# pku-lab-1806-llm/lab-1806-vec-db

Measured on AMD Instinct MI355X. Metric: queries/sec at recall@10, Gist1M d=960 (Flat brute force, L2Sqr, k=10), higher is better.
Workload: dtype f32 (int8 lower-bound filter pass); 1 GPU; flat_knn_gist1m; rows=1000000, dim=960, k=10, dist=L2Sqr, parallelism=single GPU, steps_in_flight=1, queries_per_corpus_pass=128

## Files before the change

### lab_1806_vec_db_amd/csrc/api.hip

```cpp
#include <algorithm>
#include <cmath>
#include <cstring>

#include "ctx.hpp"
#include "pq_hnsw.hpp"

using namespace vdb;

static thread_local std::string g_last_error;
void vdb::set_last_error(const std::string &m) { g_last_error = m; }
void vdb::require_gpu() {
    int cnt = 0;
    hipError_t e = hipGetDeviceCount(&cnt);
    if (e != hipSuccess || cnt <= 0)
        throw Error(VDB_ERR_NOGPU, std::string("no usable HIP device (libvdbhip has no CPU fallback): ") +
                                       hipGetErrorString(e));
}

void vdb::merge_topk_dev(Index &ix, const void *d_dists, const void *d_ids, const void *d_counts, uint64_t stride_d,
                           uint64_t stride_i, uint64_t stride_c, uint64_t n_shards, uint64_t nq, uint64_t k,
                           void *d_out_idx, void *d_out_dist, void *d_out_count, void *stream) {
    VDB_REQUIRE(d_dists && d_ids && d_counts && d_out_idx && d_out_dist && d_out_count, "null argument");
    VDB_REQUIRE(k >= 1 && k <= 1024, "k must be in 1..1024");
    VDB_REQUIRE(nq <= 65535 && n_shards <= 65535, "too many queries or shards for one call");
// ... 434 lines not shown
        ivf_set_q8((int)value);
    else if (n == "hnsw_build_gpu")
        hnsw_set_build_gpu((int)value);
    else if (n == "hnsw_pool_cap")
        hnsw_set_pool_cap((int)value);
    else if (n == "pq_adc_fast")
        pq_set_adc_fast((int)value);
    else if (n == "pq_sample16")
        pq_set_adc16_sample((int)value);
    else if (n == "pq_adc16")
        pq_set_adc16((int)value);
    else if (n == "pq_adc8_sliced")
        pq_set_adc8_sliced((int)value);
    else if (n == "flat_sample_thin")
        mfma_set_sample_thin((int)value);
    else if (n == "flat_gemm_tw")
        gemm_set_tw((int)value);
    else if (n == "flat_gemm_nt")
        gemm_set_nt((int)value);
    else if (n == "flat_gemm_zigzag")
        gemm_set_zigzag((int)value);
    else if (n == "flat_gemm_block_rows") {
        VDB_REQUIRE(value >= 0, "flat_gemm_block_rows must be >= 0");
        gemm_set_block_rows((uint64_t)value);
    }
    else if (n == "flat_gemm_stagger")
        gemm_set_stagger((int)value);
    else if (n == "flat_gemm_debug")
        idx->ix.flat_gemm_debug = (int)value;
    else if (n == "flat_tail")
        idx->ix.flat_tail_mode = (int)value;
    else if (n == "flat_tail_lb_nw")
        flat_tail_lb_set_nw((int)value);
    else if (n == "flat_small")
        idx->ix.flat_small_mode = (int)value;
    else if (n == "flat_small_max_rows")
        idx->ix.flat_small_max_rows = (uint64_t)value;
    else if (n == "flat_half")
        idx->ix.flat_half_mode = (int)value;
    else if (n == "flat_i8")
        idx->ix.flat_i8_mode = (int)value;
    else if (n == "flat_i8_rows") {
        VDB_REQUIRE(value >= 64 && value <= 8192 && value % 64 == 0, "flat_i8_rows must be a multiple of 64 in [64, 8192]");
        idx->ix.flat_i8_kprime = (uint32_t)value;
    }
    else if (n == "debug_alloc_fail_over")
        devbuf_fail_over() = (size_t)value;
    else if (n == "flat_i8_unit_min")
        idx->ix.flat_i8_unit_min = (int)value;
    else if (n == "flat_i8_full")
        idx->ix.flat_i8_full = (int)value;
    else if (n == "flat_i8_refine") {
        idx->ix.flat_i8_refine = (int)value;
        idx->ix.i8_refine_on = 0;
        idx->ix.i8_refine_calls = 0;
    }
    else if (n == "flat_i8_second")
        idx->ix.flat_i8_second = (int)value;
    else if (n == "flat_i8_stats") {
        idx->ix.flat_i8_stats = (int)value;
        for (auto &h : idx->ix.i8_rounds_hist) h = 0;
        idx->ix.i8_hits_sum = 0;
        idx->ix.i8_hits_max = 0;
        idx->ix.i8_stat_queries = 0;
    }
    else if (n == "flat_i8_hits") {
        VDB_REQUIRE(value >= 256 && value <= 4096, "flat_i8_hits must be in [256, 4096]");
        idx->ix.flat_i8_hits = (uint32_t)value;
    }
    else if (n == "flat_gemm8_sample_res")
        gemm8_set_sample_res((int)value);
    else if (n == "flat_gemm8_nt")
        gemm8_set_nt((int)value);
    else if (n == "flat_gemm8_kc")
        gemm8_set_kc((int)value);
    else if (n == "flat_gemm8_burst")
        gemm8_set_burst((int)value);
    else if (n == "flat_gemm8_res")
        gemm8_set_res((int)value);
    else if (n == "flat_gemm8_coop")
        gemm8_set_coop((int)value);
    else if (n == "flat_gemm8_grid")
        gemm8_set_grid((int)value);
    else if (n == "flat_gemm_coop")
        gemm_set_coop((int)value);
    else if (n == "flat_half_kmul") {
        VDB_REQUIRE(value >= 1 && value <= 64, "flat_half_kmul must be in [1, 64]");
        idx->ix.flat_half_kmul = (uint32_t)value;
    }
    else
        throw Error(VDB_ERR_INVALID, "unknown parameter " + n);
    VDB_API_END
}
int vdb_index_prepare(vdb_index *idx, int all_tiers) {
    VDB_API_BEGIN
    VDB_REQUIRE(idx, "null index");
    require_gpu();
// ... 15 lines not shown
        *out = idx->ix.fallback_count.load();
    else if (n == "flat_half_queries")
        *out = idx->ix.half_queries.load();
    else if (n == "flat_half_redo")
        *out = idx->ix.half_redo.load();
    else if (n == "flat_half_valid")
        *out = idx->ix.half_m.valid ? 1 : 0;
    else if (n == "flat_gemm_coop_sets")
        *out = gemm_last_coop();
    else if (n == "flat_gemm8_coop_sets")
        *out = gemm8_last_coop();
    else if (n == "flat_i8_queries")
        *out = idx->ix.i8_queries.load();
    else if (n == "flat_i8_redo")
        *out = idx->ix.i8_redo.load();
    else if (n == "flat_i8_valid")
        *out = idx->ix.i8_m.valid ? 1 : 0;
    else if (n.rfind("flat_i8_rounds_", 0) == 0 && n.size() == 16 && n[15] >= '0' && n[15] <= '8')
        *out = idx->ix.i8_rounds_hist[n[15] - '0'].load();
    else if (n == "mirror_alloc_failures")
        *out = idx->ix.mirror_alloc_failures.load();
    else if (n == "flat_i8_second_queries")
        *out = idx->ix.i8_second_queries.load();
    else if (n == "flat_i8_second_redo")
        *out = idx->ix.i8_second_redo.load();
    else if (n == "flat_i8_hits_sum")
        *out = idx->ix.i8_hits_sum.load();
    else if (n == "flat_i8_hits_max")
        *out = idx->ix.i8_hits_max.load();
    else if (n == "flat_i8_stat_queries")
        *out = idx->ix.i8_stat_queries.load();
    else if (n == "flat_i8_rows_walked")
        *out = idx->ix.i8_rows_walked.load();
    else if (n == "flat_bf16_mirror")
        *out = idx->ix.tiled_built ? 1 : 0;
    else if (n == "hnsw_heap_walk_queries")
        *out = idx->ix.hnsw.heap_walk_queries.load();
    else if (n == "hnsw_half_dropped")
        *out = idx->ix.hnsw.last_half_dropped.load();
    else if (n == "ivf_last_offers")
        *out = idx->ix.ivf.last_offers.load();
    else if (n == "ivf_last_rows_fetched_q8")
        *out = idx->ix.ivf.last_rows_fetched_q8.load();
    else if (n == "ivf_last_kept_q8")
        *out = idx->ix.ivf.last_kept_q8.load();
    else if (n == "ivf_last_kept")
        *out = idx->ix.ivf.last_kept.load();
    else if (n == "pq_adc16_queries")
        *out = idx->ix.pq.adc16_queries.load();
    else if (n == "pq_adc16_redo")
        *out = idx->ix.pq.adc16_redo.load();
    else if (n == "flat_i8_refine_queries")
        *out = idx->ix.i8_refine_queries.load();
    else if (n == "flat_i8_refine_on")
        *out = (uint64_t)idx->ix.i8_refine_on.load();
    else if (n == "pq_q8_overflow")
        *out = idx->ix.pq.q8_overflow.load();
    else if (n == "pq_q8_short")
        *out = idx->ix.pq.q8_short.load();
    else if (n == "pq_q8_hits_sum")
        *out = idx->ix.pq.q8_hits_sum.load();
    else if (n == "pq_q8_hits_max")
        *out = idx->ix.pq.q8_hits_max.load();
    else if (n == "hbm_bytes_per_row")
        *out = idx->ix.hbm_bytes_per_row();
    else
// ... 508 lines not shown
```

### lab_1806_vec_db_amd/csrc/index.hip

```cpp
#include "index.hpp"

#include <algorithm>
#include <cmath>
#include <cstring>

namespace vdb {

Index::Index(int dev, uint64_t d, int ds, bool u8) : device(dev), dim(d), dist(ds), elem_u8(u8) {
#ifndef VDB_HOST_SANITIZER_BUILD
    use_device();
    hipDeviceProp_t prop;
    VDB_HIP(hipGetDeviceProperties(&prop, dev));
    num_cu = prop.multiProcessorCount > 0 ? prop.multiProcessorCount : 256;
    std::string arch = prop.gcnArchName;
    if (arch.rfind("gfx950", 0) != 0)
        throw Error(4, "libvdbhip is built for gfx950 (MI355X) only; device reports " + arch);
#endif
}

std::unique_ptr<Workspace> Index::acquire_ws() {
    use_device();
    {
        std::lock_guard<std::mutex> g(ws_mu);
        if (!ws_free.empty()) {
// ... 564 lines not shown
            launch_mfma_pack_queries_nh(d_q, (uint32_t)nq, (uint32_t)nq_pad, (uint32_t)dim, 8, ws.qfrag_g.as<float>(), s);
        }
    }
    if (i8_second) {
        launch_i8_tau_from_dk(d_dk_hint, (uint32_t)nq, (uint32_t)nq_pad, d_qoff, ws.qsq.as<float>(), xsq_max, i8_mu_norm, (uint32_t)dim, cosine,
                              d_tau, s);
    } else {
        if (i8)
            launch_flat_gemm8_sample(d_tiled_i8.p, n, (uint32_t)dim, ws.qfrag_g.p, d_qscale, (uint32_t)ngroups, d_rowc_i8.as<float>(), s_step,
                                     ws.dense.as<float>(), ld_s, num_cu, s, unit_min ? 1 : 0);
        else if (gemm)
            launch_flat_gemm_sample(xt, n, (uint32_t)dim, ws.qfrag_g.as<float>(), d_qmul, (uint32_t)ngroups,
                                    d_sq.as<float>(), cosine, s_step, ws.dense.as<float>(), ld_s, num_cu, s);
        else
            launch_flat_mfma_sample(d_tiled.as<float>(), n, (uint32_t)dim, ws.qfrag.as<float>(), (uint32_t)nbatch,
                                    d_sq.as<float>(), cosine, s_step, ws.dense.as<float>(), ld_s, num_cu, s);
        if (n_s <= select_tau_max_n()) {
            launch_select_tau(ws.dense.as<float>(), ld_s, (uint32_t)n_s, (uint32_t)nq_pad, (uint32_t)nq, s_rank, d_tau, s);
        } else {
            const uint32_t cap_s = topk_capacity(s_rank);
            launch_topk_dense(ws.dense.as<float>(), ld_s, n_s, (uint32_t)nq_pad, s_rank, ws.lists.as<uint64_t>(), s);
            launch_topk_merge(ws.lists.as<uint64_t>(), nl_s, cap_s, (uint32_t)nq_pad, s_rank, ws.keys_a.as<uint64_t>(), s);
            launch_extract_tau(ws.keys_a.as<uint64_t>(), cap_s, (uint32_t)nq_pad, s_rank, d_tau, s);
        }
        if (nq_pad > nq && n_s > select_tau_max_n())
            VDB_HIP(hipMemsetD32Async(reinterpret_cast<hipDeviceptr_t>(d_tau + nq), (int)0xFF800000u, nq_pad - nq, s));
    }
    uint64_t *d_cand = ws.lists.as<uint64_t>();
    uint32_t *d_sync = d_hits + nq_pad;
    if (!half && !i8) VDB_HIP(hipMemsetAsync(d_hits, 0, (nq_pad + sync_words) * sizeof(uint32_t), s));
    const uint64_t hbm_passes = gemm ? ngroups : (nbatch + mfma_share() - 1) / mfma_share();
    {
        std::lock_guard<std::mutex> g(pass_mu);
        if (pass_ev_valid) VDB_HIP(hipStreamWaitEvent(s, pass_ev, 0));
    }
    prof_begin(ws, i8 ? "flat_i8" : (half ? "flat_half" : "flat_mfma"),
               double(hbm_passes) * double(n) * dim * (i8 ? 1 : (half ? sizeof(uint16_t) : sizeof(float))));
    if (i8)
        launch_flat_gemm8_filter(d_tiled_i8.p, n, (uint32_t)dim, ws.qfrag_g.p, d_qscale, (uint32_t)ngroups, d_rowc_i8.as<float>(), d_tau,
                                 d_cand, d_hits, CAND_CAP, flat_gemm_debug, num_cu, s,
                                 i8_second ? CAND_CAP : std::max<uint32_t>(64u, s_step * s_rank));
    else if (gemm)
        launch_flat_gemm_filter(xt, n, (uint32_t)dim, ws.qfrag_g.as<float>(), d_qmul, (uint32_t)ngroups,
                                d_sq.as<float>(), cosine, d_tau, d_cand, d_hits, CAND_CAP, flat_gemm_debug, num_cu, s);
    else
        launch_flat_mfma_filter(d_tiled.as<float>(), n, (uint32_t)dim, ws.qfrag.as<float>(), (uint32_t)nbatch,
                                d_sq.as<float>(), cosine, d_tau, d_cand, d_hits, CAND_CAP, d_sync, num_cu, s);
    prof_end(ws);
    {
        std::lock_guard<std::mutex> g(pass_mu);
        if (!pass_ev) VDB_HIP(hipEventCreateWithFlags(&pass_ev, hipEventDisableTiming));
        VDB_HIP(hipEventRecord(pass_ev, s));
        pass_ev_valid = true;
    }
    SplitErr se;
    if (half) {
        se.qerr = d_qerr;
        se.dx_abs = half_dx_abs;
        se.dx_rel = half_dx_rel;
    }
    if (i8) {
        se.qoff = d_qoff;
        se.mu_norm = i8_mu_norm;
    }
    if (i8 || (flat_tail_mode != 1 && !elem_u8 && flat_tail64_supported((uint32_t)dim, kprime, ksel))) {
        FlatTailArgs t{};
        t.cand = d_cand;
        t.cap = CAND_CAP;
        t.cnt = d_hits;
        t.kprime = kprime;
        t.ksel = ksel;
        t.kstride = (uint32_t)k;
        t.X = d_rows.as<float>();
        t.dim = (uint32_t)dim;
        t.Q = d_q;
        t.metric = cosine ? MET_COSINE : MET_L2_DIRECT;
        t.xsq = d_sq.as<float>();
        t.qsq = ws.qsq.as<float>();
        t.n_rows = n;
        t.xsq_max = xsq_max;
        t.xsq_min_pos = xsq_min_pos;
        t.cosine = cosine;
        t.se = se;
        t.id_offset = id_offset;
        bool refine = false;
        if (i8 && !i8_second && nq >= 64 && flat_i8_refine != 1) {
            bool on = flat_i8_refine == 2;
            if (flat_i8_refine == 0 && i8_refine_on.load() != 0) on = (i8_refine_calls.fetch_add(1) % 32u) != 31u;
            refine = on && ensure_rows_h(ws);
        }
        const size_t st_off = (nq + 15) & ~size_t(15);
        const bool want_stats = i8 && flat_i8_stats;
        t.flags = static_cast<uint8_t *>(ws.pinned(want_stats ? st_off + nq * sizeof(uint32_t) : nq));
        if (want_stats) t.qstat = reinterpret_cast<uint32_t *>(t.flags + st_off);
        p.stats = want_stats;
        p.refined = refine;
        if (refine) {
            launch_flat_refine_half(d_rows_h.as<uint16_t>(), (uint32_t)dim, half_sx(), half_dx_abs, half_dx_rel, cosine, d_q, d_sq.as<float>(),
                                    ws.qsq.as<float>(), d_qoff, d_cand, CAND_CAP, d_hits, (uint32_t)nq, CAND_CAP, s);
            i8_refine_queries += nq;
        }
        t.out_idx = d_idx;
        t.out_dist = d_dist;
        t.out_count = d_cnt;
        t.tau = d_tau;
        if (i8 && i8_second && nq <= 96 && flat_i8_full != 1) {
            ws.keys_b.reserve(nq * size_t(CAND_CAP) * sizeof(uint64_t));
            launch_flat_full_lb(t, (uint32_t)nq, ws.keys_b.as<uint64_t>(), ws.keys_c.as<uint64_t>(), s);
        } else if (i8)
            launch_flat_tail_lb(t, (uint32_t)nq, s);
        else
            launch_flat_tail64(t, (uint32_t)nq, s);
    } else {
        launch_topk_merge_counted(d_cand, CAND_CAP, d_hits, (uint32_t)nq, kprime, ws.keys_a.as<uint64_t>(), s);
        rerank_rows((uint32_t)dim, d_q, (uint32_t)nq, cosine ? MET_COSINE : MET_L2_DIRECT, d_sq.as<float>(),
                      ws.qsq.as<float>(), ws.keys_a.as<uint64_t>(), ws.keys_b.as<uint64_t>(), kprime, capp, s);
        launch_topk_merge(ws.keys_b.as<uint64_t>(), 1, capp, (uint32_t)nq, ksel, ws.keys_c.as<uint64_t>(), s);
        launch_flat_finish(ws.keys_c.as<uint64_t>(), capk, ws.keys_a.as<uint64_t>(), capp, (uint32_t)nq, ksel, (uint32_t)k, kprime,
                           n, ws.qsq.as<float>(), xsq_max, xsq_min_pos, cosine, (uint32_t)dim, se, d_hits, CAND_CAP, id_offset,
                           static_cast<uint8_t *>(ws.pinned(nq)), d_idx, d_dist, d_cnt, s);
    }
    p.active = true;
    p.half = half;
    p.i8 = i8;
    p.i8_second = i8_second;
    p.kprime = kprime;
// ... 13 lines not shown
    const uint64_t nq = p.nq, k = p.k;
    const uint8_t *flags = static_cast<const uint8_t *>(ws.pinned(nq));
    VDB_SYNC(s);
    std::vector<uint64_t> redo;
    for (uint64_t q = 0; q < nq; q++)
        if (flags[q] & 1u) redo.push_back(q);
    if (p.half) {
        half_queries += nq;
        half_redo += redo.size();
    }
    if (p.i8 && p.i8_second) {
        i8_second_queries += nq;
        i8_second_redo += redo.size();
    }
    const bool try_second = p.i8 && !p.i8_second && flat_i8_second != 1 && !redo.empty();
    if (p.i8 && !p.i8_second) {
        i8_queries += nq;
        if (!try_second) i8_redo += redo.size();
        if (flat_i8_refine == 0 && nq >= 64) {
            uint64_t rs = 0;
            for (uint64_t q = 0; q < nq; q++) rs += std::min<uint32_t>(flags[q] >> 1, 32u);
            const double mean_rounds = double(rs) / double(nq);
            if (!p.refined) {
                const int was = i8_refine_on.load();
                const int now = was ? (mean_rounds >= 4.0 ? 1 : 0) : (mean_rounds >= 6.0 ? 1 : 0);
                if (now != was) {
                    i8_refine_on = now;
                    i8_refine_calls = 0;
                }
            }
        }
        if (p.stats) {
            const uint32_t *qs = reinterpret_cast<const uint32_t *>(flags + ((nq + 15) & ~size_t(15)));
            uint64_t hs = 0, hm = 0;
            for (uint64_t q = 0; q < nq; q++) {
                const uint32_t r = qs[q] & 0xFFu, h = qs[q] >> 8;
                i8_rounds_hist[r < 8 ? r : 8] += 1;
                hs += h;
                hm = std::max<uint64_t>(hm, h);
            }
            i8_hits_sum += hs;
            i8_stat_queries += nq;
            uint64_t cur = i8_hits_max.load();
            while (hm > cur && !i8_hits_max.compare_exchange_weak(cur, hm)) {
            }
        }
    }
    if (redo.empty()) return 0;
    if (!p.half && !p.i8) fallback_count += redo.size();
    const uint64_t nr = redo.size();
    DevBuf rx, rq, rqs, ri, rd, rc, rdk;
    rx.reserve(nr * sizeof(uint64_t));
    rq.reserve(nr * dim * sizeof(float));
    rqs.reserve(nr * sizeof(float));
    ri.reserve(nr * k * sizeof(uint64_t));
    rd.reserve(nr * k * sizeof(float));
    rc.reserve(nr * sizeof(uint64_t));
    VDB_HIP(hipMemcpyAsync(rx.p, redo.data(), nr * sizeof(uint64_t), hipMemcpyHostToDevice, s));
    launch_gather_rows_f32(p.d_q, rx.as<uint64_t>(), nr, (uint32_t)dim, rq.as<float>(), s);
    launch_gather_rows_f32(ws.qsq.as<float>(), rx.as<uint64_t>(), nr, 1, rqs.as<float>(), s);
    if (try_second) {
        rdk.reserve(nr * sizeof(float));
        launch_gather_dk(p.d_dist, p.d_cnt, rx.as<uint64_t>(), nr, (uint32_t)k, p.ksel, rdk.as<float>(), s);
    }
    VDB_HIP(hipMemsetAsync(ri.p, 0, nr * k * sizeof(uint64_t), s));
    VDB_HIP(hipMemsetAsync(rd.p, 0, nr * k * sizeof(float), s));
    VDB_SYNC(s);
    if (try_second)
        i8_redo += flat_knn_device(ws, rq.as<float>(), nr, k, ri.as<uint64_t>(), rd.as<float>(), rc.as<uint64_t>(), true, 0, true, rdk.as<float>());
    else if (p.i8)
        flat_knn_device(ws, rq.as<float>(), nr, k, ri.as<uint64_t>(), rd.as<float>(), rc.as<uint64_t>(), true, 0, false);
    else if (p.half)
        flat_knn_device(ws, rq.as<float>(), nr, k, ri.as<uint64_t>(), rd.as<float>(), rc.as<uint64_t>(), false, p.kprime);
// ... 79 lines not shown
```

### lab_1806_vec_db_amd/csrc/index.hpp

```cpp
#pragma once
#include <algorithm>
#include <atomic>
#include <cmath>
#include <cstdlib>
#include <functional>
#include <map>
#include <memory>
#include <mutex>
#include <string>
#include <vector>

#include "common.hpp"
#include "kernels.hpp"

namespace vdb {

inline bool devbuf_efence() {
    static const bool on = [] {
        const char *e = std::getenv("VDB_EFENCE");
        return e && e[0] == '1';
    }();
    return on;
}
inline std::atomic<size_t> &devbuf_fail_over() {
// ... 229 lines not shown
    bool ensure_tiled(Workspace &ws);
    void prepare_flat(bool all_tiers);
    uint64_t hbm_bytes_per_row() const;
    DevBuf d_tiled_h, d_half_err;
    int half_exp = 0;
    float half_dx_abs = 0.0f, half_dx_rel = 0.0f;
    int flat_half_mode = 0;
    uint32_t flat_half_kmul = 4;
    std::atomic<uint64_t> half_queries{0}, half_redo{0};
    void half_refresh(Workspace &ws, uint64_t n_old, uint64_t n_new);
    RowMirror half_m{mirror_alloc_failures, {&d_tiled_h}};
    bool i8_defers_half() const;
    bool ensure_half(Workspace &ws);
    float half_sx() const { return std::ldexp(1.0f, 13 - half_exp); }
    DevBuf d_tiled_i8, d_rowc_i8, d_mu_i8;
    RowMirror i8_m{mirror_alloc_failures, {&d_tiled_i8, &d_rowc_i8}};
    uint64_t i8_mu_rows = 0;
    float i8_l1 = 0.0f, i8_l2 = 0.0f, i8_mu_norm = 0.0f;
    int flat_i8_mode = 0;
    uint32_t flat_i8_kprime = 2048;
    int flat_i8_full = 0;
    int flat_i8_refine = 0;
    std::atomic<int> i8_refine_on{0};
    std::atomic<uint32_t> i8_refine_calls{0};
    std::atomic<uint64_t> i8_refine_queries{0};
    int flat_i8_unit_min = 0;
    int flat_i8_second = 0;
    std::atomic<uint64_t> i8_second_queries{0}, i8_second_redo{0};
    uint32_t flat_i8_hits = 1024;
    std::atomic<uint64_t> i8_queries{0}, i8_redo{0};
    int flat_i8_stats = 0;
    std::atomic<uint64_t> i8_rounds_hist[9] = {};
    std::atomic<uint64_t> i8_hits_sum{0}, i8_hits_max{0}, i8_stat_queries{0};
    std::atomic<uint64_t> i8_rows_walked{0};
    bool i8_applicable(uint32_t ksel) const;
    bool ensure_i8(Workspace &ws);
    void build_i8(Workspace &ws);
    DevBuf d_rows_h;
    RowMirror rows_h_m{mirror_alloc_failures, {&d_rows_h}};
    int rows_h_exp = 0;
    bool ensure_rows_h(Workspace &ws);
    DevBuf d_rows_q8, d_q8_scale, d_q8_err;
    RowMirror rows_q8_m{mirror_alloc_failures, {&d_rows_q8, &d_q8_scale, &d_q8_err}};
    bool ensure_rows_q8(Workspace &ws);
    std::vector<float> h_sq;
    float xsq_max = 0.0f;
    float xsq_min_pos = 3.4e38f;
    mutable std::vector<float> h_rows;
    mutable bool host_valid = true;
    mutable std::mutex host_mu;
    int flat_mode = 0;
    int flat_gemm_mode = 0;
    int flat_gemm_debug = 0;
    int flat_tail_mode = 0;
    int flat_small_mode = 0;
    uint64_t flat_small_max_rows = 16384;
    bool flat_small_applies(uint64_t nq, uint64_t k) const;
    void flat_small_device(Workspace &ws, const float *q, uint64_t nq, uint64_t k, uint64_t *o_idx, float *o_dist, uint64_t *o_cnt);
    std::atomic<uint64_t> fallback_count{0};
    PQState pq;
    HNSWState hnsw;
    IVFState ivf;

    std::mutex ws_mu;
    std::vector<std::unique_ptr<Workspace>> ws_free;
    std::mutex pass_mu;
    hipEvent_t pass_ev = nullptr;
    bool pass_ev_valid = false;
    bool prof_on = false;
    std::mutex prof_mu;
    std::map<std::string, ProfEntry> prof;

    Index(int dev, uint64_t d, int ds, bool u8 = false);
    ~Index() {
        if (pass_ev) (void)hipEventDestroy(pass_ev);
    }
    void use_device() const {
#ifndef VDB_HOST_SANITIZER_BUILD
        VDB_HIP(hipSetDevice(device));
#endif
    }
    std::unique_ptr<Workspace> acquire_ws();
    void release_ws(std::unique_ptr<Workspace> ws);
    const float *host_rows() const;

    void add_rows(const void *rows, uint64_t count, bool on_device);
    void swap_remove(uint64_t i);

    void prof_begin(Workspace &ws, const char *name, double bytes);
    void prof_end(Workspace &ws);
    void prof_collect(Workspace &ws);

    uint64_t flat_knn_device(Workspace &ws, const float *d_q, uint64_t nq, uint64_t k, uint64_t *d_idx, float *d_dist,
                         uint64_t *d_cnt, bool allow_half = true, uint32_t kprime_min = 0, bool allow_i8 = true,
                         const float *d_dk_hint = nullptr);
    void flat_knn_enqueue(Workspace &ws, const float *d_q, uint64_t nq, uint64_t k, uint64_t *d_idx, float *d_dist, uint64_t *d_cnt,
                          bool allow_half, uint32_t kprime_min, FlatPending &p, bool allow_i8 = true, const float *d_dk_hint = nullptr);
    uint64_t flat_knn_finish(Workspace &ws, FlatPending &p);
    void flat_sorted_device(Workspace &ws, const float *d_q, uint64_t nq, uint64_t ksel, uint64_t k, uint64_t *d_idx,
                            float *d_dist, uint64_t *d_cnt);
    void scan_rows(uint64_t nrows, uint32_t d, const float *Q, uint32_t nq, int metric, const float *xsq, const float *qsq, float *out,
// ... 20 lines not shown
```

### lab_1806_vec_db_amd/csrc/k_exact.hip

```cpp
#include <algorithm>
#include <atomic>
#include <cstdio>
#include <cstdlib>
#include <vector>

#include "common.hpp"
#include "kernels.hpp"

#pragma clang fp contract(off)

namespace vdb {

enum Fold : int { FOLD_L2 = 0, FOLD_DOT = 1 };

template <int FOLD>
__device__ __forceinline__ float fold1(float acc, float x, float q) {
    if (FOLD == FOLD_L2) {
        float df = x - q;
        float sq = df * df;
        return acc + sq;
    } else {
        float p = x * q;
        return acc + p;
    }
// ... 767 lines not shown
    VDB_HIP(hipGetLastError());
}

#define TAIL_LB_AUTO_NW(nq) 40
template <int NW>
__device__ __forceinline__ uint64_t block_top64_above(const uint64_t *__restrict__ src, uint32_t total, uint64_t (*sbest)[64], uint64_t above) {
    const uint32_t lane = threadIdx.x & 63, wave = threadIdx.x >> 6;
    const uint32_t batches = (total + 255) / 256;
    uint64_t best = PAIR_NONE;
    for (uint32_t bt = wave; bt < batches; bt += NW) {
        uint64_t r[4];
#pragma unroll
        for (int u = 0; u < 4; u++) {
            const uint32_t i = (bt * 4 + u) * 64 + lane;
            const uint64_t v = i < total ? src[i] : PAIR_NONE;
            r[u] = v > above ? v : PAIR_NONE;
        }
        const uint64_t tau = __shfl(best, 63);
        uint64_t lo = r[0] < r[1] ? r[0] : r[1], lo2 = r[2] < r[3] ? r[2] : r[3];
        lo = lo < lo2 ? lo : lo2;
        if (__ballot(lo < tau) == 0) continue;
        bitonic_sort_from<2, 4>(r, lane);
        const uint64_t a = merge64(r[0], r[1], lane), b = merge64(r[2], r[3], lane);
        best = merge64(best, merge64(a, b, lane), lane);
    }
    sbest[wave][lane] = best;
    __syncthreads();
    if (wave != 0) return PAIR_NONE;
    uint64_t m = sbest[0][lane];
#pragma unroll
    for (int w = 1; w < NW; w++) m = merge64(m, sbest[w][lane], lane);
    return m;
}
__device__ __forceinline__ uint8_t flat_certify_lb(uint64_t ek, float kappa, uint32_t q, const FlatTailArgs &a) {
    if (ek == PAIR_NONE) return 1;
    const float dk = f32_from_orderable(uint32_t(ek >> 32));
    if (a.cosine) {
        const float qs = a.qsq[q], qn = sqrtf(qs);
        const bool plain = a.xsq_min_pos >= 1e-30f && qs >= 1e-30f && qs <= 1e30f && sqrtf(a.xsq_min_pos) * qn > 1e-9f;
        const float nr = 2.0f + 2.0f * a.se.mu_norm;
        float lower = 0.5f * (kappa + a.se.qoff[q]);
        lower = lower - 4.0f * 5.9604645e-8f * fabsf(lower) - float(2 * a.dim + 16) * 5.9604645e-8f * 1.01f - 2.0f * 5.9604645e-8f * nr * nr;
        return (plain && dk < lower) ? 0 : 1;
    }
    const float qn = sqrtf(a.qsq[q]);
    const float rx = fminf(sqrtf(a.xsq_max), (qn + sqrtf(fmaxf(dk, 0.0f))) * 1.001f);
    const float nr = rx + qn + 2.0f * a.se.mu_norm;
    float lower = kappa + a.se.qoff[q];
    lower = lower - float(a.dim + 8) * 5.9604645e-8f * 1.01f * fabsf(lower) - 4.0f * 5.9604645e-8f * nr * nr;
    return dk < lower ? 0 : 1;
}
template <int FOLD, int NW, int PCD>
__global__ __launch_bounds__(NW * 64, PCD ? 4 : 1) void k_flat_tail_lb(FlatTailArgs a) {
    constexpr bool PC = PCD != 0;
    static_assert(NW == 8 || NW == 4 || NW == 2 || NW == 1, "a stage covers the 64 keys of a round");
    static_assert(!PC || NW == 4, "producer / consumer fold: four waves");
    constexpr int RW = 64 / NW, NP = RW / 8;
    constexpr int DEPTH = PC ? PCD : (NW == 8 ? 8 : (NW == 4 ? 4 : (NW == 2 ? 3 : 2)));
    extern __shared__ float4 ftl_smem[];
    __shared__ uint64_t sbest[NW][64];
    __shared__ uint64_t skeys[64];
    __shared__ uint32_t s_flag;
    const uint32_t q = blockIdx.x, lane = threadIdx.x & 63, wave = threadIdx.x >> 6;
    const uint32_t d4 = a.dim / 4;
    float4 *qs4 = ftl_smem, *tile = ftl_smem + d4 + wave * (RW * 9);
    for (uint32_t i = threadIdx.x; i < d4; i += NW * 64) qs4[i] = reinterpret_cast<const float4 *>(a.Q + uint64_t(q) * a.dim)[i];
    const uint32_t cnt_q = a.cnt[q];
    const uint32_t total = cnt_q <= a.cap ? cnt_q : 0;
    const uint32_t kk = a.ksel;
    const float tau_q = a.tau[q];
    uint64_t run = PAIR_NONE;
    uint64_t above = 0;
    uint8_t flag = 1;
    const uint32_t rounds = cnt_q <= a.cap ? a.kprime / 64 : 0;
#ifdef VDB_TAIL_STAMPS
    uint32_t ns = 0;
#define TAIL_STAMP()                                                                                      \
    do {                                                                                                  \
        if (a.stamps && threadIdx.x == 0 && ns < 30) a.stamps[q * 32 + ns++] = __builtin_readcyclecounter(); \
    } while (0)
#else
#define TAIL_STAMP() do { } while (0)
#endif
    TAIL_STAMP();
    uint32_t rounds_done = 0;
    for (uint32_t rd = 0; rd < rounds; rd++) {
        rounds_done = rd + 1;
        const uint64_t best = block_top64_above<NW>(a.cand + uint64_t(q) * a.cap, total, sbest, above);
        __syncthreads();
        if (wave == 0) sbest[0][lane] = best;
        if (threadIdx.x < 64) skeys[threadIdx.x] = PAIR_NONE;
        __syncthreads();
        TAIL_STAMP();
        uint32_t idx[NP];
        bool live[NP];
#pragma unroll
        for (int i = 0; i < NP; i++) {
            const uint32_t j = wave * RW + 8 * i + (lane >> 3);
            const uint64_t c = sbest[0][j];
            live[i] = c != PAIR_NONE && j < 63;
            idx[i] = live[i] ? uint32_t(c) : 0u;
#if defined(VDB_TAIL_ABLATE) && VDB_TAIL_ABLATE == 1
            idx[i] &= 63u;
#endif
        }
        float acc;
        if constexpr (PC) {
            const bool consumer = wave == (blockIdx.x & 3u);
            acc = pc_rerank_fold<FOLD, DEPTH>(a.X, a.dim, idx, live, qs4, ftl_smem + d4, wave, lane, consumer);
            const uint64_t c = sbest[0][lane];
            if (consumer && c != PAIR_NONE && lane < 63)
                skeys[lane] = pair_key(FOLD == FOLD_L2 ? acc : epilogue(MET_COSINE, acc, a.xsq[uint32_t(c)], a.qsq[q]), uint32_t(c));
        } else {
            if constexpr (NW == 8)
                acc = group_rerank_fold<FOLD, 8>(a.X, a.dim, idx[0], live[0], qs4, tile, lane);
            else
                acc = group_rerank_fold_n<FOLD, DEPTH, RW>(a.X, a.dim, idx, live, qs4, tile, lane);
            const uint32_t j = wave * RW + lane / NW;
            const uint64_t c = sbest[0][j];
            if (c != PAIR_NONE && j < 63 && lane % NW == 0)
                skeys[j] = pair_key(FOLD == FOLD_L2 ? acc : epilogue(MET_COSINE, acc, a.xsq[uint32_t(c)], a.qsq[q]), uint32_t(c));
        }
        __syncthreads();
        TAIL_STAMP();
        if (wave == 0) {
            run = merge64(run, sort64(skeys[lane], lane), lane);
            const uint64_t ek = __shfl(run, kk - 1), nxt = sbest[0][63];
            if (lane == 0) {
                const float kappa = nxt == PAIR_NONE ? tau_q : f32_from_orderable(uint32_t(nxt >> 32));
                s_flag = flat_certify_lb(ek, kappa, q, a) | (nxt == PAIR_NONE ? 2u : 0u);
            }
        }
        __syncthreads();
        TAIL_STAMP();
        const uint32_t f = s_flag;
        if ((f & 1u) == 0) {
            flag = 0;
            break;
        }
        if (f & 2u) break;
        above = sbest[0][62];
        __syncthreads();
    }
#ifdef VDB_TAIL_STAMPS
    if (a.stamps && threadIdx.x == 0) {
        a.stamps[q * 32 + 30] = ns;
        a.stamps[q * 32 + 31] = total;
    }
#endif
    if (wave != 0) return;
    const bool ok = lane < a.ksel && run != PAIR_NONE;
    if (lane < a.ksel) {
        a.out_idx[uint64_t(q) * a.kstride + lane] = ok ? uint64_t(uint32_t(run)) + a.id_offset : 0;
        a.out_dist[uint64_t(q) * a.kstride + lane] = ok ? f32_from_orderable(uint32_t(run >> 32)) : 0.0f;
    }
    const uint32_t count = __builtin_popcountll(__ballot(ok));
    if (lane == 0) {
        if (a.out_count) a.out_count[q] = count;
        a.flags[q] = uint8_t(flag | ((rounds_done < 127u ? rounds_done : 127u) << 1));
        if (a.qstat) a.qstat[q] = rounds_done | ((cnt_q < 0xFFFFFFu ? cnt_q : 0xFFFFFFu) << 8);
    }
}
bool flat_tail_lb_supported(uint32_t dim, uint32_t kprime, uint32_t ksel) {
    return (dim & 3) == 0 && dim >= 64 && dim <= 8192 && kprime >= 64 && kprime % 64 == 0 && kprime <= 8192 && ksel >= 1 && ksel <= 64;
}
static std::atomic<int> g_tail_lb_nw{0};
void flat_tail_lb_set_nw(int v) { g_tail_lb_nw = v; }
#ifdef VDB_TAIL_STAMPS
static void tail_stamps_report(unsigned long long *d, uint32_t nq, hipStream_t s) {
    VDB_SYNC(s);
    std::vector<unsigned long long> h(size_t(nq) * 32);
    VDB_HIP(hipMemcpy(h.data(), d, h.size() * 8, hipMemcpyDeviceToHost));
    VDB_HIP(hipFree(d));
    uint32_t hist[8] = {0}, nr = 0;
    double sel = 0, fold = 0, cert = 0, life = 0;
    for (uint32_t q = 0; q < nq; q++) {
        const unsigned long long *t = &h[size_t(q) * 32];
        const uint32_t ns = (uint32_t)t[30], r = ns ? (ns - 1) / 3 : 0;
        hist[r < 7 ? r : 7]++;
        if (ns) life += double(t[ns - 1] - t[0]);
        for (uint32_t i = 0; i < r; i++, nr++) {
            sel += double(t[1 + 3 * i] - t[3 * i]);
            fold += double(t[2 + 3 * i] - t[1 + 3 * i]);
            cert += double(t[3 + 3 * i] - t[2 + 3 * i]);
        }
    }
    fprintf(stderr, "TAIL_STAMPS nq %u  queries by rounds 0:%u 1:%u 2:%u 3:%u 4:%u 5+:%u  ticks per round: select %.0f fold %.0f merge+certify %.0f  per workgroup %.0f\n",
            nq, hist[0], hist[1], hist[2], hist[3], hist[4], hist[5] + hist[6] + hist[7], sel / (nr ? nr : 1), fold / (nr ? nr : 1),
            cert / (nr ? nr : 1), life / nq);
}
#endif
void launch_flat_tail_lb(const FlatTailArgs &a0, uint32_t nq, hipStream_t s) {
    if (nq == 0) return;
    FlatTailArgs a = a0;
#ifdef VDB_TAIL_STAMPS
    static std::atomic<int> calls{0};
    const char *want = getenv("VDB_TAIL_STAMPS");
    unsigned long long *stamps = nullptr;
    if (want && ++calls == atoi(want)) {
        VDB_HIP(hipMalloc(&stamps, size_t(nq) * 32 * 8));
        VDB_HIP(hipMemset(stamps, 0, size_t(nq) * 32 * 8));
        a.stamps = stamps;
    }
#endif
    VDB_REQUIRE(flat_tail_lb_supported(a.dim, a.kprime, a.ksel) && (a.metric == MET_L2_DIRECT || a.metric == MET_COSINE) && a.se.qoff && a.tau,
                "flat_tail_lb: unsupported shape");
    VDB_REQUIRE((a.metric == MET_COSINE) == (a.cosine != 0) && (a.metric == MET_L2_DIRECT || (a.xsq && a.qsq)), "flat_tail_lb: metric / norms");
    const size_t lds = (size_t(a.dim / 4) + 2 * 64 * 9) * sizeof(float4);
    int nw = g_tail_lb_nw;
    if (nw != 8 && nw != 4 && nw != 2 && nw != 1 && nw != 40 && nw != 41) nw = TAIL_LB_AUTO_NW(nq);
    if (a.metric == MET_COSINE) {
        if (nw == 8)
            hipLaunchKernelGGL((k_flat_tail_lb<FOLD_DOT, 8, 0>), dim3(nq), dim3(512), lds, s, a);
        else if (nw == 41)
            hipLaunchKernelGGL((k_flat_tail_lb<FOLD_DOT, 4, 5>), dim3(nq), dim3(256), lds, s, a);
        else
            hipLaunchKernelGGL((k_flat_tail_lb<FOLD_DOT, 4, 3>), dim3(nq), dim3(256), lds, s, a);
    } else if (nw == 40)
        hipLaunchKernelGGL((k_flat_tail_lb<FOLD_L2, 4, 3>), dim3(nq), dim3(256), lds, s, a);
    else if (nw == 41)
        hipLaunchKernelGGL((k_flat_tail_lb<FOLD_L2, 4, 5>), dim3(nq), dim3(256), lds, s, a);
    else if (nw == 8)
        hipLaunchKernelGGL((k_flat_tail_lb<FOLD_L2, 8, 0>), dim3(nq), dim3(512), lds, s, a);
    else if (nw == 4)
        hipLaunchKernelGGL((k_flat_tail_lb<FOLD_L2, 4, 0>), dim3(nq), dim3(256), lds, s, a);
    else if (nw == 2)
        hipLaunchKernelGGL((k_flat_tail_lb<FOLD_L2, 2, 0>), dim3(nq), dim3(128), lds, s, a);
// ... 47 lines not shown
```

### lab_1806_vec_db_amd/csrc/kernels.hpp

```cpp
#pragma once
#include <hip/hip_runtime.h>

#include <cstdint>

namespace vdb {

enum Metric : int {
    MET_L2_DIRECT = 0,
    MET_COSINE = 1,
    MET_L2_CACHED = 2,
};

void launch_row_sqnorm(const float *X, uint64_t n, uint32_t dim, float *sq, hipStream_t s);
void launch_scan_exact(const float *X, uint64_t n, uint32_t dim, const float *Q, uint32_t nq, int metric,
                       const float *xsq, const float *qsq, float *out, uint64_t ld, bool use_lds, hipStream_t s);
void launch_rerank(const float *X, uint32_t dim, const float *Q, uint32_t nq, int metric, const float *xsq,
                   const float *qsq, const uint64_t *cand, uint64_t *out, uint32_t ncand, uint32_t ldc,
                   hipStream_t s, const uint32_t *cnt = nullptr);
void launch_finalize(const uint64_t *keys, uint32_t ldk, uint32_t nq, uint32_t ksel, uint32_t kstride,
                     uint64_t id_offset, uint64_t *out_idx, float *out_dist, uint64_t *out_count, hipStream_t s);
void launch_iota_keys(uint64_t *rows, uint32_t nq, uint32_t n, uint32_t ld, hipStream_t s);
struct SplitErr {
    const float *qerr = nullptr;
    float dx_abs = 0.0f, dx_rel = 0.0f;
    const float *qoff = nullptr;
    float mu_norm = 0.0f;
};
void launch_flat_finish(const uint64_t *exact_sorted, uint32_t lde, const uint64_t *approx_sorted, uint32_t lda,
                        uint32_t nq, uint32_t ksel, uint32_t kstride, uint32_t kprime, uint64_t n_rows, const float *qsq,
                        float xsq_max, float xsq_min_pos, int cosine, uint32_t dim, SplitErr se, const uint32_t *cnt, uint32_t cap,
                        uint64_t id_offset, uint8_t *flags, uint64_t *out_idx, float *out_dist, uint64_t *out_count,
                        hipStream_t s);
struct FlatTailArgs {
    const uint64_t *cand;
    uint32_t cap;
    const uint32_t *cnt;
    uint32_t kprime, ksel, kstride;
    const float *X;
    uint32_t dim;
    const float *Q;
    int metric;
    const float *xsq, *qsq;
    uint64_t n_rows;
    float xsq_max, xsq_min_pos;
    int cosine;
    SplitErr se;
    uint64_t id_offset;
    uint8_t *flags;
    uint64_t *out_idx;
    float *out_dist;
    uint64_t *out_count;
    unsigned long long *stamps = nullptr;
    const float *tau = nullptr;
    uint32_t *qstat = nullptr;
};
bool flat_tail_lb_supported(uint32_t dim, uint32_t kprime, uint32_t ksel);
void launch_flat_tail_lb(const FlatTailArgs &a, uint32_t nq, hipStream_t s);
void launch_flat_full_lb(const FlatTailArgs &a, uint32_t nq, uint64_t *exact_keys, uint64_t *topk, hipStream_t s);
void flat_tail_lb_set_nw(int v);
bool flat_tail64_supported(uint32_t dim, uint32_t kprime, uint32_t ksel);
void launch_flat_tail64(const FlatTailArgs &a, uint32_t nq, hipStream_t s);
struct FlatSmallArgs {
    const float *X;
    uint64_t n;
    uint32_t dim;
    const float *Q;
    int metric;
    const float *xsq;
    uint64_t *part;
    uint32_t *counter;
    uint32_t ksel, kstride;
    uint64_t id_offset;
    uint64_t *out_idx;
    float *out_dist;
    uint64_t *out_count;
};
bool flat_small_supported(uint64_t n, uint32_t dim, uint64_t nq, uint64_t k);
uint32_t flat_small_rows_per_wg(uint64_t n, int num_cu);
size_t flat_small_part_keys(uint64_t n, uint64_t nq, uint32_t ksel, int num_cu);
void launch_flat_small(const FlatSmallArgs &a, uint32_t nq, int num_cu, hipStream_t s);
void launch_certify(const uint64_t *exact_sorted, uint32_t lde, const uint64_t *approx_sorted, uint32_t lda,
                    uint32_t nq, uint32_t k, uint32_t kprime, uint64_t n_rows, const float *qsq, float xsq_max,
                    float xsq_min_pos, int cosine, uint32_t dim, uint8_t *flags, hipStream_t s);

void launch_extract_tau(const uint64_t *sorted, uint32_t ld, uint32_t nq, uint32_t kprime, float *tau, hipStream_t s);
void launch_flag_overflow(const uint32_t *cnt, uint32_t cap, uint32_t min_hits, uint32_t nq, uint8_t *flags,
                          hipStream_t s);

uint32_t topk_chunk(uint64_t n);
uint32_t topk_num_lists(uint64_t n);
void launch_select_tau(const float *keys, uint64_t ld, uint32_t n, uint32_t nq, uint32_t nq_real, uint32_t kth, float *tau,
                       hipStream_t s);
// ... 127 lines not shown
```

Measured before the change: 1.056 million queries/s.

## Cut tail rerank rounds at certified bound and cache live candidate list

```diff
diff --git a/lab_1806_vec_db_amd/csrc/api.hip b/lab_1806_vec_db_amd/csrc/api.hip
--- a/lab_1806_vec_db_amd/csrc/api.hip
+++ b/lab_1806_vec_db_amd/csrc/api.hip
@@ -490,6 +490,10 @@
         idx->ix.flat_tail_mode = (int)value;
     else if (n == "flat_tail_lb_nw")
         flat_tail_lb_set_nw((int)value);
+    else if (n == "flat_tail_cut")
+        flat_tail_lb_set_cut((int)value);
+    else if (n == "flat_pass_wait")
+        idx->ix.flat_pass_wait = (int)value;
     else if (n == "flat_small")
         idx->ix.flat_small_mode = (int)value;
     else if (n == "flat_small_max_rows")
@@ -521,6 +525,8 @@
         idx->ix.i8_hits_sum = 0;
         idx->ix.i8_hits_max = 0;
         idx->ix.i8_stat_queries = 0;
+        idx->ix.i8_rows_walked = 0;
+        idx->ix.i8_rows_fetched = 0;
     }
     else if (n == "flat_i8_hits") {
         VDB_REQUIRE(value >= 256 && value <= 4096, "flat_i8_hits must be in [256, 4096]");
@@ -602,6 +608,8 @@
         *out = idx->ix.i8_stat_queries.load();
     else if (n == "flat_i8_rows_walked")
         *out = idx->ix.i8_rows_walked.load();
+    else if (n == "flat_i8_rows_fetched")
+        *out = idx->ix.i8_rows_fetched.load();
     else if (n == "flat_bf16_mirror")
         *out = idx->ix.tiled_built ? 1 : 0;
     else if (n == "hnsw_heap_walk_queries")
diff --git a/lab_1806_vec_db_amd/csrc/index.hip b/lab_1806_vec_db_amd/csrc/index.hip
--- a/lab_1806_vec_db_amd/csrc/index.hip
+++ b/lab_1806_vec_db_amd/csrc/index.hip
@@ -620,7 +620,7 @@
     const uint64_t hbm_passes = gemm ? ngroups : (nbatch + mfma_share() - 1) / mfma_share();
     {
         std::lock_guard<std::mutex> g(pass_mu);
-        if (pass_ev_valid) VDB_HIP(hipStreamWaitEvent(s, pass_ev, 0));
+        if (pass_ev_valid && (pass_ev_stream != s || flat_pass_wait == 1)) VDB_HIP(hipStreamWaitEvent(s, pass_ev, 0));
     }
     prof_begin(ws, i8 ? "flat_i8" : (half ? "flat_half" : "flat_mfma"),
                double(hbm_passes) * double(n) * dim * (i8 ? 1 : (half ? sizeof(uint16_t) : sizeof(float))));
@@ -639,6 +639,7 @@
         std::lock_guard<std::mutex> g(pass_mu);
         if (!pass_ev) VDB_HIP(hipEventCreateWithFlags(&pass_ev, hipEventDisableTiming));
         VDB_HIP(hipEventRecord(pass_ev, s));
+        pass_ev_stream = s;
         pass_ev_valid = true;
     }
     SplitErr se;
@@ -679,7 +680,7 @@
         }
         const size_t st_off = (nq + 15) & ~size_t(15);
         const bool want_stats = i8 && flat_i8_stats;
-        t.flags = static_cast<uint8_t *>(ws.pinned(want_stats ? st_off + nq * sizeof(uint32_t) : nq));
+        t.flags = static_cast<uint8_t *>(ws.pinned(want_stats ? st_off + 2 * nq * sizeof(uint32_t) : nq));
         if (want_stats) t.qstat = reinterpret_cast<uint32_t *>(t.flags + st_off);
         p.stats = want_stats;
         p.refined = refine;
@@ -759,13 +760,17 @@
         }
         if (p.stats) {
             const uint32_t *qs = reinterpret_cast<const uint32_t *>(flags + ((nq + 15) & ~size_t(15)));
-            uint64_t hs = 0, hm = 0;
+            uint64_t hs = 0, hm = 0, rf = 0, rw = 0;
             for (uint64_t q = 0; q < nq; q++) {
                 const uint32_t r = qs[q] & 0xFFu, h = qs[q] >> 8;
                 i8_rounds_hist[r < 8 ? r : 8] += 1;
                 hs += h;
                 hm = std::max<uint64_t>(hm, h);
+                rf += qs[nq + q] & 0xFFFFu;
+                rw += qs[nq + q] >> 16;
             }
+            i8_rows_fetched += rf;
+            i8_rows_walked += rw;
             i8_hits_sum += hs;
             i8_stat_queries += nq;
             uint64_t cur = i8_hits_max.load();
diff --git a/lab_1806_vec_db_amd/csrc/index.hpp b/lab_1806_vec_db_amd/csrc/index.hpp
--- a/lab_1806_vec_db_amd/csrc/index.hpp
+++ b/lab_1806_vec_db_amd/csrc/index.hpp
@@ -285,7 +285,7 @@
     int flat_i8_stats = 0;
     std::atomic<uint64_t> i8_rounds_hist[9] = {};
     std::atomic<uint64_t> i8_hits_sum{0}, i8_hits_max{0}, i8_stat_queries{0};
-    std::atomic<uint64_t> i8_rows_walked{0};
+    std::atomic<uint64_t> i8_rows_walked{0}, i8_rows_fetched{0};
     bool i8_applicable(uint32_t ksel) const;
     bool ensure_i8(Workspace &ws);
     void build_i8(Workspace &ws);
@@ -320,6 +320,8 @@
     std::mutex pass_mu;
     hipEvent_t pass_ev = nullptr;
     bool pass_ev_valid = false;
+    hipStream_t pass_ev_stream = nullptr;
+    int flat_pass_wait = 0;
     bool prof_on = false;
     std::mutex prof_mu;
     std::map<std::string, ProfEntry> prof;
diff --git a/lab_1806_vec_db_amd/csrc/k_exact.hip b/lab_1806_vec_db_amd/csrc/k_exact.hip
--- a/lab_1806_vec_db_amd/csrc/k_exact.hip
+++ b/lab_1806_vec_db_amd/csrc/k_exact.hip
@@ -823,26 +823,136 @@
     for (int w = 1; w < NW; w++) m = merge64(m, sbest[w][lane], lane);
     return m;
 }
-__device__ __forceinline__ uint8_t flat_certify_lb(uint64_t ek, float kappa, uint32_t q, const FlatTailArgs &a) {
-    if (ek == PAIR_NONE) return 1;
-    const float dk = f32_from_orderable(uint32_t(ek >> 32));
+struct FlatCertTerms {
+    bool none, cosine, plain;
+    float dk, qoff, rel, abs2;
+};
+__device__ __forceinline__ FlatCertTerms flat_certify_terms(uint64_t ek, uint32_t q, const FlatTailArgs &a) {
+    FlatCertTerms t;
+    t.none = ek == PAIR_NONE;
+    t.cosine = a.cosine != 0;
+    t.plain = true;
+    t.dk = f32_from_orderable(uint32_t(ek >> 32));
+    t.qoff = t.rel = t.abs2 = 0.0f;
+    if (t.none) return t;
+    t.qoff = a.se.qoff[q];
     if (a.cosine) {
         const float qs = a.qsq[q], qn = sqrtf(qs);
-        const bool plain = a.xsq_min_pos >= 1e-30f && qs >= 1e-30f && qs <= 1e30f && sqrtf(a.xsq_min_pos) * qn > 1e-9f;
+        t.plain = a.xsq_min_pos >= 1e-30f && qs >= 1e-30f && qs <= 1e30f && sqrtf(a.xsq_min_pos) * qn > 1e-9f;
         const float nr = 2.0f + 2.0f * a.se.mu_norm;
-        float lower = 0.5f * (kappa + a.se.qoff[q]);
-        lower = lower - 4.0f * 5.9604645e-8f * fabsf(lower) - float(2 * a.dim + 16) * 5.9604645e-8f * 1.01f - 2.0f * 5.9604645e-8f * nr * nr;
-        return (plain && dk < lower) ? 0 : 1;
+        t.rel = float(2 * a.dim + 16) * 5.9604645e-8f * 1.01f;
+        t.abs2 = 2.0f * 5.9604645e-8f * nr * nr;
+        return t;
     }
     const float qn = sqrtf(a.qsq[q]);
-    const float rx = fminf(sqrtf(a.xsq_max), (qn + sqrtf(fmaxf(dk, 0.0f))) * 1.001f);
+    const float rx = fminf(sqrtf(a.xsq_max), (qn + sqrtf(fmaxf(t.dk, 0.0f))) * 1.001f);
     const float nr = rx + qn + 2.0f * a.se.mu_norm;
-    float lower = kappa + a.se.qoff[q];
-    lower = lower - float(a.dim + 8) * 5.9604645e-8f * 1.01f * fabsf(lower) - 4.0f * 5.9604645e-8f * nr * nr;
-    return dk < lower ? 0 : 1;
+    t.rel = float(a.dim + 8) * 5.9604645e-8f * 1.01f;
+    t.abs2 = 4.0f * 5.9604645e-8f * nr * nr;
+    return t;
+}
+__device__ __forceinline__ uint8_t flat_certify_eval(const FlatCertTerms &t, float kappa) {
+    if (t.none) return 1;
+    if (t.cosine) {
+        float lower = 0.5f * (kappa + t.qoff);
+        lower = lower - 4.0f * 5.9604645e-8f * fabsf(lower) - t.rel - t.abs2;
+        return (t.plain && t.dk < lower) ? 0 : 1;
+    }
+    float lower = kappa + t.qoff;
+    lower = lower - t.rel * fabsf(lower) - t.abs2;
+    return t.dk < lower ? 0 : 1;
+}
+__device__ __forceinline__ uint8_t flat_certify_lb(uint64_t ek, float kappa, uint32_t q, const FlatTailArgs &a) {
+    return flat_certify_eval(flat_certify_terms(ek, q, a), kappa);
+}
+__device__ __forceinline__ void sort256(uint64_t (&r)[4], uint32_t lane) {
+    bitonic_sort_from<2, 4>(r, lane);
+    {
+        const uint64_t v1 = lane_reverse64(r[1], lane), v3 = lane_reverse64(r[3], lane);
+        const uint64_t a = r[0], b = r[2];
+        r[0] = a < v1 ? a : v1;
+        r[1] = a < v1 ? v1 : a;
+        r[2] = b < v3 ? b : v3;
+        r[3] = b < v3 ? v3 : b;
+        bitonic_stages<64, 32, 4>(r, lane);
+    }
+    const uint64_t s2 = lane_reverse64(r[3], lane), s3 = lane_reverse64(r[2], lane);
+    const uint64_t l0 = r[0] < s2 ? r[0] : s2, h0 = r[0] < s2 ? s2 : r[0], l1 = r[1] < s3 ? r[1] : s3, h1 = r[1] < s3 ? s3 : r[1];
+    r[0] = l0 < l1 ? l0 : l1;
+    r[1] = l0 < l1 ? l1 : l0;
+    r[2] = h0 < h1 ? h0 : h1;
+    r[3] = h0 < h1 ? h1 : h0;
+    bitonic_stages<64, 32, 4>(r, lane);
+}
+constexpr uint32_t TAIL_LIVE_MAX = 255;
+template <int NW>
+__device__ __forceinline__ bool tail_live_list(const uint64_t *__restrict__ src, uint32_t total, uint64_t above, uint64_t ek, uint32_t q,
+                                               const FlatTailArgs &a, uint64_t *slive , uint32_t *s_n, uint64_t *s_kmin) {
+    const uint32_t lane = threadIdx.x & 63, wave = threadIdx.x >> 6;
+    if (threadIdx.x == 0) {
+        *s_n = 0;
+        *s_kmin = PAIR_NONE;
+    }
+    __syncthreads();
+    uint64_t kmin = PAIR_NONE;
+    const FlatCertTerms terms = flat_certify_terms(ek, q, a);
+    constexpr int CH = 8;
+    for (uint32_t i0 = wave * 64; i0 < total; i0 += NW * 64 * CH) {
+        uint64_t vs[CH];
+#pragma unroll
+        for (int c = 0; c < CH; c++) {
+            const uint32_t i = i0 + c * NW * 64 + lane;
+            vs[c] = i < total ? src[i] : PAIR_NONE;
+        }
+#pragma unroll
+        for (int c = 0; c < CH; c++) {
+            if (i0 + c * NW * 64 >= total) break;
+            const uint64_t v = vs[c];
+            const bool in = v != PAIR_NONE && v > above;
+            const bool cert = in && flat_certify_eval(terms, f32_from_orderable(uint32_t(v >> 32))) == 0;
+            if (cert && v < kmin) kmin = v;
+            const bool keep = in && !cert;
+            const unsigned long long m = __ballot(keep);
+            if (m) {
+                uint32_t base = 0;
+                if (lane == 0) base = atomicAdd(s_n, uint32_t(__builtin_popcountll(m)));
+                base = __shfl(base, 0);
+                const uint32_t slot = base + uint32_t(__builtin_popcountll(m & ((1ull << lane) - 1ull)));
+                if (keep && slot < 256) slive[slot] = v;
+            }
+        }
+    }
+#pragma unroll
+    for (int o = 32; o >= 1; o >>= 1) {
+        const uint64_t t = __shfl_xor(kmin, o);
+        kmin = t < kmin ? t : kmin;
+    }
+    if (lane == 0 && kmin != PAIR_NONE) atomicMin(reinterpret_cast<unsigned long long *>(s_kmin), (unsigned long long)kmin);
+    __syncthreads();
+    const uint32_t n = *s_n;
+    if (n > TAIL_LIVE_MAX) return false;
+    if (wave == 0) {
+        if (n <= 64) {
+            const uint64_t v = sort64(lane < n ? slive[lane] : PAIR_NONE, lane);
+            slive[lane] = v;
+#pragma unroll
+            for (int u = 1; u < 4; u++) slive[u * 64 + lane] = PAIR_NONE;
+        } else {
+            uint64_t r[4];
+#pragma unroll
+            for (int u = 0; u < 4; u++) r[u] = u * 64 + lane < n ? slive[u * 64 + lane] : PAIR_NONE;
+            sort256(r, lane);
+#pragma unroll
+            for (int u = 0; u < 4; u++) slive[u * 64 + lane] = r[u];
+        }
+        slive[256 + lane] = PAIR_NONE;
+        if (lane == 0) slive[n] = *s_kmin;
+    }
+    __syncthreads();
+    return true;
 }
 template <int FOLD, int NW, int PCD>
-__global__ __launch_bounds__(NW * 64, PCD ? 4 : 1) void k_flat_tail_lb(FlatTailArgs a) {
+__global__ __launch_bounds__(NW * 64, (PCD || NW == 4) ? 4 : 1) void k_flat_tail_lb(FlatTailArgs a) {
     constexpr bool PC = PCD != 0;
     static_assert(NW == 8 || NW == 4 || NW == 2 || NW == 1, "a stage covers the 64 keys of a round");
     static_assert(!PC || NW == 4, "producer / consumer fold: four waves");
@@ -851,7 +961,8 @@
     extern __shared__ float4 ftl_smem[];
     __shared__ uint64_t sbest[NW][64];
     __shared__ uint64_t skeys[64];
-    __shared__ uint32_t s_flag;
+    __shared__ uint32_t s_flag, s_cut, s_nlive;
+    __shared__ uint64_t slive[320], s_ek, s_kmin;
     const uint32_t q = blockIdx.x, lane = threadIdx.x & 63, wave = threadIdx.x >> 6;
     const uint32_t d4 = a.dim / 4;
     float4 *qs4 = ftl_smem, *tile = ftl_smem + d4 + wave * (RW * 9);
@@ -874,22 +985,45 @@
 #define TAIL_STAMP() do { } while (0)
 #endif
     TAIL_STAMP();
-    uint32_t rounds_done = 0;
+    uint32_t rounds_done = 0, fetched = 0;
+    bool tried = false, have_list = false;
+    uint32_t cur = 0, walked = 0;
     for (uint32_t rd = 0; rd < rounds; rd++) {
         rounds_done = rd + 1;
-        const uint64_t best = block_top64_above<NW>(a.cand + uint64_t(q) * a.cap, total, sbest, above);
-        __syncthreads();
-        if (wave == 0) sbest[0][lane] = best;
+        if (a.cut && rd != 0 && !tried && s_ek != PAIR_NONE) {
+            tried = true;
+            have_list = tail_live_list<NW>(a.cand + uint64_t(q) * a.cap, total, above, s_ek, q, a, slive, &s_nlive, &s_kmin);
+            cur = 0;
+        }
+        if (have_list && cur > 256) have_list = false;
+        uint64_t best;
+        if (have_list) {
+            best = wave == 0 ? slive[cur + lane] : PAIR_NONE;
+        } else {
+            best = block_top64_above<NW>(a.cand + uint64_t(q) * a.cap, total, sbest, above);
+            __syncthreads();
+        }
+        if (wave == 0) {
+            sbest[0][lane] = best;
+            if (a.cut && rd != 0) {
+                const uint64_t ek = __shfl(run, kk - 1);
+                const bool cert = ek != PAIR_NONE && best != PAIR_NONE && flat_certify_lb(ek, f32_from_orderable(uint32_t(best >> 32)), q, a) == 0;
+                const unsigned long long m = __ballot(cert);
+                if (lane == 0) s_cut = m ? uint32_t(__builtin_ctzll(m)) : 64u;
+            } else if (lane == 0)
+                s_cut = 64u;
+        }
         if (threadIdx.x < 64) skeys[threadIdx.x] = PAIR_NONE;
         __syncthreads();
         TAIL_STAMP();
+        const uint32_t stop = s_cut < 63u ? s_cut : 63u;
         uint32_t idx[NP];
         bool live[NP];
 #pragma unroll
         for (int i = 0; i < NP; i++) {
             const uint32_t j = wave * RW + 8 * i + (lane >> 3);
             const uint64_t c = sbest[0][j];
-            live[i] = c != PAIR_NONE && j < 63;
+            live[i] = c != PAIR_NONE && j < stop;
             idx[i] = live[i] ? uint32_t(c) : 0u;
 #if defined(VDB_TAIL_ABLATE) && VDB_TAIL_ABLATE == 1
             idx[i] &= 63u;
@@ -900,7 +1034,7 @@
             const bool consumer = wave == (blockIdx.x & 3u);
             acc = pc_rerank_fold<FOLD, DEPTH>(a.X, a.dim, idx, live, qs4, ftl_smem + d4, wave, lane, consumer);
             const uint64_t c = sbest[0][lane];
-            if (consumer && c != PAIR_NONE && lane < 63)
+            if (consumer && c != PAIR_NONE && lane < stop)
                 skeys[lane] = pair_key(FOLD == FOLD_L2 ? acc : epilogue(MET_COSINE, acc, a.xsq[uint32_t(c)], a.qsq[q]), uint32_t(c));
         } else {
             if constexpr (NW == 8)
@@ -909,15 +1043,19 @@
                 acc = group_rerank_fold_n<FOLD, DEPTH, RW>(a.X, a.dim, idx, live, qs4, tile, lane);
             const uint32_t j = wave * RW + lane / NW;
             const uint64_t c = sbest[0][j];
-            if (c != PAIR_NONE && j < 63 && lane % NW == 0)
+            if (c != PAIR_NONE && j < stop && lane % NW == 0)
                 skeys[j] = pair_key(FOLD == FOLD_L2 ? acc : epilogue(MET_COSINE, acc, a.xsq[uint32_t(c)], a.qsq[q]), uint32_t(c));
         }
         __syncthreads();
         TAIL_STAMP();
         if (wave == 0) {
             run = merge64(run, sort64(skeys[lane], lane), lane);
-            const uint64_t ek = __shfl(run, kk - 1), nxt = sbest[0][63];
+            const uint64_t ek = __shfl(run, kk - 1), nxt = sbest[0][stop];
+            if (a.qstat)
+                fetched += uint32_t(__builtin_popcountll(__ballot(lane < stop && sbest[0][lane] != PAIR_NONE))) +
+                           ((total - walked < 63u ? total - walked : 63u) << 16);
             if (lane == 0) {
+                s_ek = ek;
                 const float kappa = nxt == PAIR_NONE ? tau_q : f32_from_orderable(uint32_t(nxt >> 32));
                 s_flag = flat_certify_lb(ek, kappa, q, a) | (nxt == PAIR_NONE ? 2u : 0u);
             }
@@ -930,7 +1068,9 @@
             break;
         }
         if (f & 2u) break;
-        above = sbest[0][62];
+        if (stop != 0) above = sbest[0][stop - 1];
+        cur += stop;
+        walked += stop;
         __syncthreads();
     }
 #ifdef VDB_TAIL_STAMPS
@@ -949,7 +1089,10 @@
     if (lane == 0) {
         if (a.out_count) a.out_count[q] = count;
         a.flags[q] = uint8_t(flag | ((rounds_done < 127u ? rounds_done : 127u) << 1));
-        if (a.qstat) a.qstat[q] = rounds_done | ((cnt_q < 0xFFFFFFu ? cnt_q : 0xFFFFFFu) << 8);
+        if (a.qstat) {
+            a.qstat[q] = rounds_done | ((cnt_q < 0xFFFFFFu ? cnt_q : 0xFFFFFFu) << 8);
+            a.qstat[a.nq + q] = fetched;
+        }
     }
 }
 bool flat_tail_lb_supported(uint32_t dim, uint32_t kprime, uint32_t ksel) {
@@ -957,6 +1100,8 @@
 }
 static std::atomic<int> g_tail_lb_nw{0};
 void flat_tail_lb_set_nw(int v) { g_tail_lb_nw = v; }
+static std::atomic<int> g_tail_lb_cut{0};
+void flat_tail_lb_set_cut(int v) { g_tail_lb_cut = v; }
 #ifdef VDB_TAIL_STAMPS
 static void tail_stamps_report(unsigned long long *d, uint32_t nq, hipStream_t s) {
     VDB_SYNC(s);
@@ -976,6 +1121,28 @@
             cert += double(t[3 + 3 * i] - t[2 + 3 * i]);
         }
     }
+    double rs[4] = {0}, rf[4] = {0}, rc[4] = {0}, lf[5] = {0}, lmax = 0;
+    uint32_t rn[4] = {0}, ln[5] = {0};
+    for (uint32_t q = 0; q < nq; q++) {
+        const unsigned long long *t = &h[size_t(q) * 32];
+        const uint32_t ns = (uint32_t)t[30], r = ns ? (ns - 1) / 3 : 0;
+        if (!ns) continue;
+        const double l = double(t[ns - 1] - t[0]);
+        lf[r < 4 ? r : 4] += l;
+        ln[r < 4 ? r : 4]++;
+        lmax = l > lmax ? l : lmax;
+        for (uint32_t i = 0; i < r; i++) {
+            const uint32_t j = i < 3 ? i : 3;
+            rs[j] += double(t[1 + 3 * i] - t[3 * i]);
+            rf[j] += double(t[2 + 3 * i] - t[1 + 3 * i]);
+            rc[j] += double(t[3 + 3 * i] - t[2 + 3 * i]);
+            rn[j]++;
+        }
+    }
+    for (int j = 0; j < 4; j++)
+        if (rn[j]) fprintf(stderr, "TAIL_STAMPS   round %d%s (%u): select %.0f fold %.0f merge+certify %.0f\n", j + 1, j == 3 ? "+" : "", rn[j], rs[j] / rn[j], rf[j] / rn[j], rc[j] / rn[j]);
+    fprintf(stderr, "TAIL_STAMPS   ticks per workgroup by rounds walked 1: %.0f 2: %.0f 3: %.0f 4+: %.0f  longest %.0f\n", ln[1] ? lf[1] / ln[1] : 0.0,
+            ln[2] ? lf[2] / ln[2] : 0.0, ln[3] ? lf[3] / ln[3] : 0.0, ln[4] ? lf[4] / ln[4] : 0.0, lmax);
     fprintf(stderr, "TAIL_STAMPS nq %u  queries by rounds 0:%u 1:%u 2:%u 3:%u 4:%u 5+:%u  ticks per round: select %.0f fold %.0f merge+certify %.0f  per workgroup %.0f\n",
             nq, hist[0], hist[1], hist[2], hist[3], hist[4], hist[5] + hist[6] + hist[7], sel / (nr ? nr : 1), fold / (nr ? nr : 1),
             cert / (nr ? nr : 1), life / nq);
@@ -984,6 +1151,8 @@
 void launch_flat_tail_lb(const FlatTailArgs &a0, uint32_t nq, hipStream_t s) {
     if (nq == 0) return;
     FlatTailArgs a = a0;
+    a.cut = g_tail_lb_cut == 1 ? 0 : 1;
+    a.nq = nq;
 #ifdef VDB_TAIL_STAMPS
     static std::atomic<int> calls{0};
     const char *want = getenv("VDB_TAIL_STAMPS");
diff --git a/lab_1806_vec_db_amd/csrc/kernels.hpp b/lab_1806_vec_db_amd/csrc/kernels.hpp
--- a/lab_1806_vec_db_amd/csrc/kernels.hpp
+++ b/lab_1806_vec_db_amd/csrc/kernels.hpp
@@ -53,11 +53,14 @@
     unsigned long long *stamps = nullptr;
     const float *tau = nullptr;
     uint32_t *qstat = nullptr;
+    uint32_t nq = 0;
+    int cut = 0;
 };
 bool flat_tail_lb_supported(uint32_t dim, uint32_t kprime, uint32_t ksel);
 void launch_flat_tail_lb(const FlatTailArgs &a, uint32_t nq, hipStream_t s);
 void launch_flat_full_lb(const FlatTailArgs &a, uint32_t nq, uint64_t *exact_keys, uint64_t *topk, hipStream_t s);
 void flat_tail_lb_set_nw(int v);
+void flat_tail_lb_set_cut(int v);
 bool flat_tail64_supported(uint32_t dim, uint32_t kprime, uint32_t ksel);
 void launch_flat_tail64(const FlatTailArgs &a, uint32_t nq, hipStream_t s);
 struct FlatSmallArgs {
```

New measurement: 1.066 million queries/s (median of 6 runs). 1.01x the previous value.
